# IST-DASLab/torch_cgx

Hardware: AMD Instinct MI355X
Metric: DDP samples/sec ResNet-50 4-bit (higher is better)
Workload: dtype bf16; 1 GPU; model=resnet50, global_batch=256, input=3x224x224, parallelism=dp1, backend=cgx, bits=4, bucket_size=1024, compression_active=False

## Files before the change

csrc/bindings.cc:

```cpp
#include <torch/extension.h>

#include <ATen/hip/impl/HIPStreamMasqueradingAsCUDA.h>
#include <torch/csrc/utils/pybind.h>

#include <ATen/hip/impl/HIPGuardImplMasqueradingAsCUDA.h>

#include <cstring>
#include <functional>
#include <thread>
#include <tuple>

#include "backend.h"
#include "bn_plan.h"
#include "collectives.h"
#include "conv1x1_plan.h"
#include "reducer.h"

namespace cgx {
namespace {

void run_rank_threads(int ws, int dev,
                      const std::function<void(int, hipStream_t)>& body,
                      const std::function<void()>& abort) {
  std::vector<hipStream_t> qs(ws, nullptr);
// ... 810 lines not shown
  for (int wg = 0; wg < p.grid; wg++)
    for (int tid = 0; tid < kBnThreads; tid++) {
      const BnSweep sw = bn_sweep(p, wg, tid);
      int64_t k = 0;
      for (int64_t r = sw.row; r < p.rows; r += sw.stride, k++) {
        TORCH_CHECK(k < width, "bn_sweep_indices: run longer than planned");
        o[((int64_t)wg * kBnThreads + tid) * width + k] = bn_vec(p, r, sw.cg);
      }
    }
  return out;
}

std::vector<int64_t> py_bn_partial_offsets(int64_t rows, int64_t channels,
                                           int wg) {
  const BnPlan p = bn_plan(rows, channels);
  TORCH_CHECK(p.eligible && wg >= 0 && wg < p.grid, "bn_partial_offsets: bad");
  std::vector<int64_t> offs;
  for (int tid = 0; tid < p.tc; tid++) {
    const BnSweep sw = bn_sweep(p, wg, tid);
    const int64_t o = bn_partial_offset(p, wg, sw.cg);
    for (int j = 0; j < 8; j++) offs.push_back(o + j);
  }
  return offs;
}


Conv1x1Plan conv1x1_plan_of(const at::Tensor& x, const at::Tensor& weight,
                            int64_t max_workgroups) {
  return conv1x1_plan(x.numel() / x.size(1), x.size(1), weight.size(0),
                      (int)std::min<int64_t>(max_workgroups, 1 << 20));
}

bool py_conv1x1_eligible(const at::Tensor& x, const at::Tensor& weight) {
  return bn_tensor_ok(x) && weight.is_cuda() &&
         weight.device() == x.device() &&
         weight.scalar_type() == at::kBFloat16 && weight.dim() == 4 &&
         weight.size(1) == x.size(1) && weight.size(2) == 1 &&
         weight.size(3) == 1 && weight.is_contiguous() &&
         reinterpret_cast<uintptr_t>(weight.data_ptr()) % 16 == 0 &&
         conv1x1_plan_of(x, weight, 0).eligible;
}

std::tuple<at::Tensor, at::Tensor> py_conv1x1_stats(const at::Tensor& x,
                                                    const at::Tensor& weight,
                                                    int64_t max_workgroups) {
  TORCH_CHECK(max_workgroups >= 0, "conv1x1_stats: max_workgroups >= 0");
  TORCH_CHECK(py_conv1x1_eligible(x, weight),
              "conv1x1_stats: input or weight is not eligible");
  const Conv1x1Plan p = conv1x1_plan_of(x, weight, max_workgroups);
  c10::hip::HIPGuardMasqueradingAsCUDA guard(x.device().index());
  auto y = at::empty({x.size(0), p.n, x.size(2), x.size(3)}, x.options(),
                     at::MemoryFormat::ChannelsLast);
  auto part = at::empty({p.splits, p.pstride}, x.options().dtype(at::kFloat));
  launch_conv1x1_stats(p, x.data_ptr(), weight.data_ptr(), y.data_ptr(),
                       part.data_ptr<float>(), bn_stream(x));
  return {y, part};
}

py::dict py_conv1x1_plan(int64_t rows, int64_t k, int64_t n,
                         int64_t max_workgroups) {
  const Conv1x1Plan p = conv1x1_plan(rows, k, n, (int)max_workgroups);
  py::dict d;
  d["eligible"] = p.eligible;
  d["native"] = p.native;
  d["threads"] = kConvThreads;
  d["tile_rows"] = kConvTileRows;
  d["mfma_tiles"] = p.nt;
  d["tile_channels"] = p.bn;
  d["ntiles"] = p.ntiles;
  d["k_chunk"] = p.kc;
  d["k_chunks"] = p.nchunks;
  d["resident"] = p.resident;
  d["row_tiles"] = p.row_tiles;
  d["splits"] = p.splits;
  d["grid"] = p.grid;
  d["tiles_per_split"] = p.tiles_per_split;
  d["run"] = p.run;
  d["lds_bytes"] = p.lds_bytes;
  d["partial_stride"] = p.pstride;
  d["partial_floats"] = p.partial_floats;
  return d;
}

at::Tensor py_conv1x1_walk(int64_t rows, int64_t k, int64_t n,
                           int64_t max_workgroups) {
  const Conv1x1Plan p = conv1x1_plan(rows, k, n, (int)max_workgroups);
  TORCH_CHECK(p.eligible, "conv1x1_walk: shape is not eligible");
  auto out = at::full({p.grid, p.tiles_per_split, 4}, -1,
                      at::TensorOptions().dtype(at::kLong));
  int64_t* o = out.data_ptr<int64_t>();
  for (int wg = 0; wg < p.grid; wg++) {
    const int split = conv1x1_split(p, wg), nt = conv1x1_ntile(p, wg);
    for (int i = 0; i < p.tiles_per_split; i++) {
      const int t = conv1x1_tile(p, split, i);
      if (t >= p.row_tiles) break;
      int64_t* e = o + ((int64_t)wg * p.tiles_per_split + i) * 4;
      e[0] = (int64_t)t * kConvTileRows;
      e[1] = std::min<int64_t>(e[0] + kConvTileRows, p.rows);
      e[2] = (int64_t)nt * p.bn;
      e[3] = e[2] + p.bn;
    }
  }
  return out;
}

void py_register_layer(int64_t bucket_idx, int64_t layer_idx, int64_t numel,
                       int64_t bits, int64_t bucket_size) {
  Registry::get().register_layer((int)bucket_idx, (int)layer_idx, numel,
                                 (int)bits, (int)bucket_size);
}

void py_set_bits(int64_t bucket_idx, int64_t layer_idx, int64_t bits) {
  Registry::get().set_bits((int)bucket_idx, (int)layer_idx, (int)bits);
}

void py_set_bucket(int64_t bucket_idx, int64_t layer_idx,
                   int64_t bucket_size) {
  Registry::get().set_bucket_size((int)bucket_idx, (int)layer_idx,
                                  (int)bucket_size);
}

}
}

PYBIND11_MODULE(TORCH_EXTENSION_NAME, m) {
  py::class_<cgx::ProcessGroupCGX,
             c10::intrusive_ptr<cgx::ProcessGroupCGX>, c10d::Backend>(
      m, "ProcessGroupCGX")
      .def(py::init<c10::intrusive_ptr<c10d::Store>, int, int,
                    c10::intrusive_ptr<c10d::Backend>>(),
           py::arg("store"), py::arg("rank"), py::arg("size"),
           py::arg("cpu_delegate") = nullptr);

  m.def("register_layer", &cgx::py_register_layer, py::arg("bucket_idx"),
        py::arg("layer_idx"), py::arg("layer_numel"), py::arg("bits"),
        py::arg("bucket_size"));
  m.def("set_quantization_bits", &cgx::py_set_bits);
  m.def("set_quantization_bucket_size", &cgx::py_set_bucket);
  m.def("clear_registry", [] { cgx::Registry::get().clear(); });
  m.def("registry_match",
        [](int64_t numel, int64_t key) {
          cgx::Registry::BucketInfo info;
          const bool ok = cgx::Registry::get().next(
              numel, reinterpret_cast<const void*>(key), &info);
          return py::make_tuple(ok, ok ? info.idx : -1);
        },
        py::arg("numel"), py::arg("key") = 0);
  m.def("registry_snapshot", [] {
    py::list out;
    auto& reg = cgx::Registry::get();
    for (const auto& b : reg.snapshot()) {
      py::list numels, cfgs;
      for (auto n : b.numels) numels.append(n);
      for (const auto& c : b.cfgs)
        cfgs.append(py::make_tuple(c.bits, c.bucket_size));
      out.append(py::make_tuple(b.idx, numels, cfgs));
    }
    return out;
  });

  m.def("parse_engine_config", [] {
    auto c = cgx::EngineConfig::from_env();
    py::dict d;
    d["fusion_bytes"] = c.fusion_bytes;
    d["min_elems"] = c.min_elems;
    d["default_bits"] = c.default_bits;
    d["default_bucket"] = c.default_bucket;
    d["stochastic"] = c.stochastic;
    d["inner_ring"] = c.ring;
    d["cross_ring"] = c.cross_ring;
    d["debug_a2a"] = c.debug_a2a;
    d["fake_ratio"] = c.fake_ratio;
    d["skip_incomplete"] = c.skip_incomplete;
    d["dummy"] = c.dummy;
    d["intra_compress"] = c.intra_compress;
    d["intra_broadcast"] = c.intra_broadcast;
    d["error_feedback"] = c.error_feedback;
    return d;
  });
  m.def("env_flag", &cgx::env_flag, py::arg("name"),
        py::arg("default") = false,
        "Test seam: the textual boolean parser (only \"0\" is false).");
  m.def("env_int", &cgx::env_int, py::arg("name"), py::arg("default"),
        "Test seam: the numeric parser behind the `!= 0` booleans.");
  m.def("loopback_allreduce", &cgx::py_loopback_allreduce, py::arg("buckets"),
        "Run Reducer::allreduce (flat) at world_size=len(buckets) on one GPU "
// ... 31 lines not shown
        py::arg("skip_incomplete") = false);
  m.def("dequantize_multi", &cgx::py_dequantize_multi, py::arg("comp"),
        py::arg("out"), py::arg("bits"), py::arg("bucket_size"),
        py::arg("add") = false);
  m.def("compute_topology",
        [](const c10::intrusive_ptr<c10d::Store>& store, int rank, int size,
           const std::string& hostname) {
          auto t = cgx::compute_topology(store, rank, size, hostname);
          return std::make_tuple(t.node_id, t.local_rank, t.local_size,
                                 t.n_nodes, t.uniform);
        },
        "Exchange hostnames through the store -> (node_id, local_rank, "
        "local_size, n_nodes, uniform)");
  m.def("buffer_size", &cgx::py_buffer_size, py::arg("n"), py::arg("dtype"),
        py::arg("bits"), py::arg("bucket_size"),
        py::arg("skip_incomplete") = false);
  m.def("partition", &cgx::py_partition);
  m.def("plan_bucket", &cgx::py_plan_bucket, py::arg("layer_numels"),
        py::arg("layer_cfgs"), py::arg("dtype"), py::arg("fusion_bytes"),
        py::arg("min_elems"), py::arg("fake_ratio") = 1.0,
        py::arg("dummy") = false,
        "Test seam: the bucket plan for layers laid out back to back from "
        "byte offset 0 -> (uncomp [(byte_off, count)], chunks [[(byte_off, "
        "numel, bits, bucket)]]).");
  m.def("plan_chunk", &cgx::py_plan_chunk, py::arg("views"), py::arg("dtype"),
        py::arg("ws"), py::arg("skip_incomplete") = false,
        "Test seam: the rank plan of one chunk [(byte_off, numel, bits, "
        "bucket)] -> (offs, szs, comp, rs [[(byte_off, n, bits, bucket, "
        "comp_off, skip_incomplete, fb_off)]]).");
  m.def("route_quantize", &cgx::py_route_quantize, py::arg("slices"),
        "Test seam: the launch router's quantize plan for "
        "[(in, out, fb, n, bits, bucket, skip_incomplete)] (pointers as "
        "ints) -> [(bits, kind, descs, cum, any_residual, max_gpl)].");
  m.def("route_dequantize", &cgx::py_route_dequantize, py::arg("slices"),
        py::arg("dtype"), py::arg("src_stride") = 0, py::arg("nsrc") = 1,
        py::arg("add") = false,
        "Test seam: the launch router's dequantize plan for "
        "[(in, out, n, bits, bucket, skip_incomplete)] -> "
        "[(bits, kind, descs, total_groups, any_residual)].");
  m.def("bn_act_forward", &cgx::py_bn_act_forward, py::arg("x"),
        py::arg("identity"), py::arg("weight"), py::arg("bias"),
        py::arg("running_mean"), py::arg("running_var"), py::arg("momentum"),
        py::arg("eps"), py::arg("relu"), py::arg("part") = py::none(),
        "Training-mode BatchNorm2d of a channels_last bf16 tensor, fused with "
        "an optional residual add and ReLU -> (out, mean, invstd, mask | "
        "None); updates the running statistics in place.  With `part`, the "
        "partials conv1x1_stats returned with x, the statistics pass over x "
        "is skipped.");
  m.def("bn_act_backward", &cgx::py_bn_act_backward, py::arg("dy"),
        py::arg("x"), py::arg("mean"), py::arg("invstd"), py::arg("weight"),
        py::arg("mask"), py::arg("has_identity"),
        "Backward of bn_act_forward -> (dx, dgamma, dbeta, didentity | None).");
  m.def("bn_act2_forward", &cgx::py_bn_act2_forward, py::arg("x3"),
        py::arg("xd"), py::arg("weight3"), py::arg("bias3"),
        py::arg("running_mean3"), py::arg("running_var3"),
        py::arg("momentum3"), py::arg("eps3"), py::arg("weightd"),
        py::arg("biasd"), py::arg("running_meand"), py::arg("running_vard"),
        py::arg("momentumd"), py::arg("epsd"), py::arg("relu"),
        py::arg("part3") = py::none(), py::arg("partd") = py::none(),
        "relu(bn3(x3) + bn_d(xd)) with both BatchNorms in training mode: "
        "(x3, xd, weight3, bias3, running_mean3, running_var3, momentum3, "
        "eps3, weightd, biasd, running_meand, running_vard, momentumd, epsd, "
        "relu, part3=None, partd=None) -> (out, mean3, invstd3, meand, "
        "invstdd, mask | None); part3 / partd as `part` of bn_act_forward.");
  m.def("conv1x1_stats", &cgx::py_conv1x1_stats, py::arg("x"),
        py::arg("weight"), py::arg("max_workgroups") = 0,
        "conv2d(x, weight) of a 1x1 / stride 1 / no-bias convolution on a "
        "channels_last bf16 tensor -> (y, part); part holds the per-channel "
        "(count, mean, M2) partials of y.  max_workgroups > 0 caps the "
        "persistent grid.");
  m.def("conv1x1_eligible", &cgx::py_conv1x1_eligible, py::arg("x"),
        py::arg("weight"),
        "True where conv1x1_stats takes (x, weight): CUDA, bf16, dense "
        "channels_last input, [N, K, 1, 1] weight, and a shape conv1x1_plan "
        "calls eligible.");
  m.def("conv1x1_plan", &cgx::py_conv1x1_plan, py::arg("rows"), py::arg("k"),
        py::arg("n"), py::arg("max_workgroups") = 0,
        "The launch geometry of conv1x1_stats for [rows, k] x [n, k], and "
        "`native`: whether the model uses it at this shape.");
  m.def("conv1x1_walk", &cgx::py_conv1x1_walk, py::arg("rows"), py::arg("k"),
        py::arg("n"), py::arg("max_workgroups") = 0,
        "Test seam: [grid, tiles_per_split, 4] int64, (row0, row1, n0, n1) "
        "of every tile each workgroup visits (-1: none).");
  m.def("bn_act2_backward", &cgx::py_bn_act2_backward,
        "Backward of bn_act2_forward: (dy, x3, xd, mean3, invstd3, weight3, "
        "meand, invstdd, weightd, mask) -> (dx3, dxd, dgamma3, dbeta3, "
        "dgammad, dbetad).");
  m.def("bn_act_pool_forward", &cgx::py_bn_act_pool_forward, py::arg("x"),
        py::arg("weight"), py::arg("bias"), py::arg("running_mean"),
        py::arg("running_var"), py::arg("momentum"), py::arg("eps"),
        "max_pool2d(relu(bn(x)), 3, 2, 1) in training mode -> (pooled, mean, "
        "invstd, arg); arg is one byte per pooled element.");
  m.def("bn_act_pool_backward", &cgx::py_bn_act_pool_backward, py::arg("dy"),
        py::arg("x"), py::arg("mean"), py::arg("invstd"), py::arg("weight"),
        py::arg("arg"),
        "Backward of bn_act_pool_forward -> (dx, dgamma, dbeta).");
  m.def("bn_pool_geometry", &cgx::py_bn_pool_geometry, py::arg("h"),
        py::arg("w"),
        "Test seam: (windows [oh*ow, 9], covers [h*w, 4, 2]) of the stem's "
        "3x3/2/1 pooling as the kernels index it.");
  m.def("bn_eligible", &cgx::py_bn_eligible, py::arg("x"),
        "True where the fused BatchNorm kernels take `x`: CUDA, bf16, dense "
        "channels_last, and a shape bn_plan calls eligible.");
  m.def("bn_plan", &cgx::py_bn_plan, py::arg("rows"), py::arg("channels"),
        "Test seam: the launch geometry of the fused BatchNorm kernels for a "
        "[rows, channels] activation.");
  m.def("bn_sweep_indices", &cgx::py_bn_sweep_indices, py::arg("rows"),
        py::arg("channels"),
        "Test seam: [grid*threads, rows_per_thread+1] int64, the 16-byte "
        "vector indices every thread visits (-1: none).");
  m.def("bn_partial_offsets", &cgx::py_bn_partial_offsets, py::arg("rows"),
        py::arg("channels"), py::arg("wg"),
        "Test seam: the partial-buffer floats workgroup `wg` writes.");
  m.attr("FLAG_SKIP_INCOMPLETE") = cgx::kFlagSkipIncomplete;
  m.attr("FLAG_TAIL_ONLY") = cgx::kFlagTailOnly;
  m.attr("KIND_FAST") = (int)cgx::kFast;
  m.attr("KIND_GENERIC") = (int)cgx::kGeneric;
  m.attr("KIND_TWO_PASS") = (int)cgx::kTwoPass;
  m.attr("KIND_SUB") = (int)cgx::kSub;
}
```

csrc/conv1x1_kernels.hip:

```cpp
#include <hip/hip_runtime.h>

#include "bn_moments.h"
#include "check.h"
#include "conv1x1_plan.h"

namespace cgx {
namespace {

constexpr int kT = kConvThreads;

typedef __bf16 bf16x8 __attribute__((ext_vector_type(8)));
typedef __bf16 bf16x2 __attribute__((ext_vector_type(2)));
typedef float f32x2 __attribute__((ext_vector_type(2)));
typedef float f32x16 __attribute__((ext_vector_type(16)));

template <int KC>
__device__ inline int w_slot(int n, int q) {
  return n * (KC / 8) + (q ^ (KC == 64 ? (n >> 1) & 7 : n & 15));
}

__device__ inline int acc_row(int i, int h) {
  return (i & 3) + 8 * (i >> 2) + 4 * h;
}

// ... 105 lines not shown
      if (acc_row(2 * e + 1, h) < live) st.push(hi);
    }

    const int odd = c & 1;
#pragma unroll
    for (int jp = 0; jp < NT / 2; jp++) {
#pragma unroll
      for (int jj = 0; jj < 2; jj++)
#pragma unroll
        for (int e = 0; e < 8; e++) {
          const unsigned own = pk[2 * jp + jj][e];
          const unsigned other = (unsigned)__builtin_amdgcn_update_dpp(
              0, (int)own, 0xB1, 0xf, 0xf, false);
          const unsigned word = odd ? (other >> 16) | (own & 0xffff0000u)
                                    : (own & 0xffffu) | (other << 16);
          const int row = acc_row(2 * e, h) + odd;
          stage32[row * 32 + ((jj * 16 + (c >> 1)) ^ ((row & 1) << 4))] = word;
        }
      asm volatile("" ::: "memory");
      __builtin_amdgcn_wave_barrier();
#pragma unroll
      for (int u = 0; u < 4; u++) {
        const int idx = u * 64 + lane, row = idx >> 3, q = idx & 7;
        const uint4 v = stage[row * 8 + (q ^ ((row & 1) << 2))];
        if (row < live) y[(r0 + row) * nvec + (n0 + jp * 64) / 8 + q] = v;
      }
      asm volatile("" ::: "memory");
      __builtin_amdgcn_wave_barrier();
    }
  }

  __syncthreads();
  float* sc = reinterpret_cast<float*>(lds);
  const int run = wave * 2 + h;
#pragma unroll
  for (int j = 0; j < NT; j++) {
    sc[run * BN + j * 32 + c] = st.mean[j];
    sc[(8 + run) * BN + j * 32 + c] = st.m2[j];
  }
  if (c == 0) sc[16 * BN + run] = st.n;
  __syncthreads();
  if (tid < BN) {
    Moments<1> m[8];
#pragma unroll
    for (int r = 0; r < 8; r++) {
      m[r].n = sc[16 * BN + r];
      m[r].mean[0] = sc[r * BN + tid];
      m[r].m2[0] = sc[(8 + r) * BN + tid];
    }
#pragma unroll
    for (int step = 1; step < 8; step *= 2)
#pragma unroll
      for (int r = 0; r < 8; r += 2 * step)
        m[r].merge(m[r + step].n, m[r + step].mean, m[r + step].m2);
    float* row = part + (int64_t)split * p.pstride;
    row[n0 + tid] = m[0].mean[0];
    row[p.n + n0 + tid] = m[0].m2[0];
    if (tid == 0) row[2 * p.n + ntile] = m[0].n;
  }
}

template <int NT, int KC, bool RES>
void launch(const Conv1x1Plan& p, const void* x, const void* w, void* y,
            float* part, hipStream_t stream) {
  static const hipError_t attr = hipFuncSetAttribute(
      reinterpret_cast<const void*>(&conv1x1_stats<NT, KC, RES>),
      hipFuncAttributeMaxDynamicSharedMemorySize,
      kConvWLdsBytes + kConvStageBytes);
  CGX_HIP_CHECK(attr);
  hipLaunchKernelGGL((conv1x1_stats<NT, KC, RES>), dim3(p.grid), dim3(kT),
                     p.lds_bytes, stream, static_cast<const uint4*>(x),
                     static_cast<const uint4*>(w), static_cast<uint4*>(y), part,
                     p);
}

template <int NT>
void launch_nt(const Conv1x1Plan& p, const void* x, const void* w, void* y,
               float* part, hipStream_t stream) {
  if (p.kc == 64) launch<NT, 64, true>(p, x, w, y, part, stream);
  else if (p.resident) launch<NT, 128, true>(p, x, w, y, part, stream);
  else launch<NT, 128, false>(p, x, w, y, part, stream);
}

}

void launch_conv1x1_stats(const Conv1x1Plan& p, const void* x, const void* w,
                          void* y, float* part, hipStream_t stream) {
  TORCH_CHECK(p.eligible, "conv1x1_stats: shape is not eligible");
  if (p.nt == 2) launch_nt<2>(p, x, w, y, part, stream);
  else if (p.nt == 4) launch_nt<4>(p, x, w, y, part, stream);
  else launch_nt<8>(p, x, w, y, part, stream);
  CGX_HIP_CHECK(hipGetLastError());
}

}
```

csrc/conv1x1_plan.cc:

```cpp
#include "conv1x1_plan.h"

#include <algorithm>

namespace cgx {
namespace {

struct Measured {
  int k, n;
  int64_t rows;
};
constexpr Measured kNative[] = {
    {64, 64, 802816},   {64, 256, 802816},  {256, 64, 802816},
    {256, 128, 802816}, {128, 512, 200704}, {512, 128, 200704},
    {256, 1024, 50176},
};

bool measured_faster(int64_t rows, int k, int n) {
  for (const Measured& m : kNative)
    if (m.k == k && m.n == n && m.rows == rows) return true;
  return false;
}

bool pow2_in(int64_t v, int64_t lo, int64_t hi) {
  return v >= lo && v <= hi && (v & (v - 1)) == 0;
}

}

Conv1x1Plan conv1x1_plan(int64_t rows, int64_t k, int64_t n,
                         int max_workgroups) {
  Conv1x1Plan p;
  p.rows = rows;
  p.eligible = pow2_in(k, 64, 2048) && pow2_in(n, 64, 2048) && rows >= 2 &&
               rows <= kBnMaxRows;
  if (!p.eligible) return p;
  p.k = (int)k;
  p.n = (int)n;
  p.native = measured_faster(rows, p.k, p.n);

  p.nt = std::min(p.n / 32, kConvMaxNt);
  p.bn = 32 * p.nt;
  p.ntiles = p.n / p.bn;
  p.kc = p.k == 64 ? 64 : 128;
  p.nchunks = p.k / p.kc;
  p.resident = p.bn * p.k * 2 <= kConvWLdsBytes;
  p.lds_bytes = p.bn * (p.resident ? p.k : p.kc) * 2 + kConvStageBytes;

  p.row_tiles = (int)((rows + kConvTileRows - 1) / kConvTileRows);
  const int by_regs = p.nt == 8 ? 1 : p.nt == 4 ? 2 : 3;
  const int per_cu = std::max(1, std::min(kConvLdsBytes / p.lds_bytes, by_regs));
  int64_t splits = std::min<int64_t>(
      p.row_tiles, std::max(1, kConvCus * per_cu / p.ntiles));
  splits = std::min(splits, std::max<int64_t>(1, rows / 82));
  if (max_workgroups > 0)
    splits = std::min<int64_t>(splits, std::max(1, max_workgroups / p.ntiles));
  p.splits = (int)splits;
  p.grid = p.ntiles * p.splits;
  p.tiles_per_split = (p.row_tiles + p.splits - 1) / p.splits;
  p.run = 16 * p.tiles_per_split;
  p.pstride = 2 * p.n + p.ntiles;
  p.partial_floats = (int64_t)p.splits * p.pstride;
  return p;
}

}
```

csrc/conv1x1_plan.h:

```cpp
#pragma once

#include <cstdint>

#include "bn_plan.h"

namespace cgx {

constexpr int kConvThreads = 256;
constexpr int kConvTileRows = 128;
constexpr int kConvMaxNt = 8;
constexpr int kConvCus = 256;
constexpr int kConvLdsBytes = 160 * 1024;
constexpr int kConvWLdsBytes = 128 * 1024;
constexpr int kConvStageBytes = 16 * 1024;

struct Conv1x1Plan {
  int64_t rows = 0;
  int k = 0, n = 0;
  bool eligible = false;
  bool native = false;
  int nt = 0;
  int bn = 0;
  int ntiles = 0;
  int kc = 0;
  int nchunks = 0;
  bool resident = false;
  int row_tiles = 0;
  int splits = 0;
  int grid = 0;
  int tiles_per_split = 0;
  int run = 0;
  int lds_bytes = 0;
  int pstride = 0;
  int64_t partial_floats = 0;
};

Conv1x1Plan conv1x1_plan(int64_t rows, int64_t k, int64_t n,
                         int max_workgroups = 0);

__host__ __device__ inline int conv1x1_ntile(const Conv1x1Plan& p, int wg) {
  return wg % p.ntiles;
}
__host__ __device__ inline int conv1x1_split(const Conv1x1Plan& p, int wg) {
  return wg / p.ntiles;
}
__host__ __device__ inline int conv1x1_tile(const Conv1x1Plan& p, int split,
                                            int i) {
  return split + i * p.splits;
}

inline BnPartials conv1x1_partials(const float* part, int n, int splits,
                                   int ntiles) {
  BnPartials q;
  q.mean = part;
  q.m2 = part + n;
  q.cnt = part + 2 * n;
  q.channels = n;
  q.splits = splits;
  q.tc = n / ntiles / 8;
  q.pstride = q.cstride = 2 * n + ntiles;
  return q;
}

void launch_conv1x1_stats(const Conv1x1Plan& p, const void* x, const void* w,
                          void* y, float* part, hipStream_t stream);

}
```

torch_cgx_amd/models/resnet.py:

```python

from __future__ import annotations

import torch
import torch.nn as nn

from ..ops.fused_bn import bn_act, bn_act_pool, conv_bn_act


class Bottleneck(nn.Module):
    expansion = 4

    def __init__(self, inplanes: int, planes: int, stride: int = 1,
                 downsample: nn.Module = None):
        super().__init__()
        self.conv1 = nn.Conv2d(inplanes, planes, 1, bias=False)
        self.bn1 = nn.BatchNorm2d(planes)
        self.conv2 = nn.Conv2d(planes, planes, 3, stride=stride, padding=1,
                               bias=False)
        self.bn2 = nn.BatchNorm2d(planes)
        self.conv3 = nn.Conv2d(planes, planes * self.expansion, 1, bias=False)
        self.bn3 = nn.BatchNorm2d(planes * self.expansion)
        self.relu = nn.ReLU(inplace=True)
        self.downsample = downsample
        self.stride = stride

    def forward(self, x):
        identity = x
        out = conv_bn_act(self.conv1, self.bn1, x)
        out = bn_act(self.bn2, self.conv2(out))
        if self.downsample is not None:
            conv, bn = self.downsample[0], self.downsample[1]
            return conv_bn_act(self.conv3, self.bn3, out, identity,
                               identity_conv=conv, identity_bn=bn)
        return conv_bn_act(self.conv3, self.bn3, out, identity)


class ResNet(nn.Module):
    def __init__(self, layers, num_classes: int = 1000):
        super().__init__()
        self.inplanes = 64
        self.conv1 = nn.Conv2d(3, 64, 7, stride=2, padding=3, bias=False)
        self.bn1 = nn.BatchNorm2d(64)
        self.relu = nn.ReLU(inplace=True)
        self.maxpool = nn.MaxPool2d(3, stride=2, padding=1)
        self.layer1 = self._make_layer(64, layers[0])
        self.layer2 = self._make_layer(128, layers[1], stride=2)
        self.layer3 = self._make_layer(256, layers[2], stride=2)
        self.layer4 = self._make_layer(512, layers[3], stride=2)
        self.avgpool = nn.AdaptiveAvgPool2d(1)
        self.fc = nn.Linear(512 * Bottleneck.expansion, num_classes)
        for m in self.modules():
            if isinstance(m, nn.Conv2d):
                nn.init.kaiming_normal_(m.weight, mode="fan_out",
                                        nonlinearity="relu")
            elif isinstance(m, nn.BatchNorm2d):
                nn.init.constant_(m.weight, 1)
                nn.init.constant_(m.bias, 0)

    def _make_layer(self, planes: int, blocks: int, stride: int = 1):
        downsample = None
        if stride != 1 or self.inplanes != planes * Bottleneck.expansion:
            downsample = nn.Sequential(
                nn.Conv2d(self.inplanes, planes * Bottleneck.expansion, 1,
                          stride=stride, bias=False),
                nn.BatchNorm2d(planes * Bottleneck.expansion),
            )
        layers = [Bottleneck(self.inplanes, planes, stride, downsample)]
        self.inplanes = planes * Bottleneck.expansion
        for _ in range(1, blocks):
            layers.append(Bottleneck(self.inplanes, planes))
        return nn.Sequential(*layers)

    def forward(self, x):
        x = bn_act_pool(self.bn1, self.conv1(x), self.maxpool)
        x = self.layer4(self.layer3(self.layer2(self.layer1(x))))
        x = self.avgpool(x).flatten(1)
        return self.fc(x)


def resnet50(num_classes: int = 1000) -> ResNet:
    return ResNet([3, 4, 6, 3], num_classes)


def resnet18(num_classes: int = 1000) -> nn.Module:

    class BasicBlock(nn.Module):
        def __init__(self, inp, planes, stride=1, down=None):
            super().__init__()
            self.c1 = nn.Conv2d(inp, planes, 3, stride, 1, bias=False)
            self.b1 = nn.BatchNorm2d(planes)
            self.c2 = nn.Conv2d(planes, planes, 3, 1, 1, bias=False)
            self.b2 = nn.BatchNorm2d(planes)
            self.down = down

        def forward(self, x):
            idt = x if self.down is None else self.down(x)
            out = torch.relu(self.b1(self.c1(x)))
            return torch.relu(self.b2(self.c2(out)) + idt)

    class R18(nn.Module):
        def __init__(self):
            super().__init__()
            self.stem = nn.Sequential(
                nn.Conv2d(3, 64, 7, 2, 3, bias=False), nn.BatchNorm2d(64),
                nn.ReLU(inplace=True), nn.MaxPool2d(3, 2, 1))
            chans = [64, 128, 256, 512]
            blocks = []
            inp = 64
            for i, c in enumerate(chans):
                stride = 1 if i == 0 else 2
                down = None
# ... 17 lines not shown
```

torch_cgx_amd/ops/fused_bn.py:

```python

from __future__ import annotations

import os

import torch
import torch.nn.functional as F

from .. import _C


class _BnAct(torch.autograd.Function):
    @staticmethod
    def forward(ctx, x, identity, weight, bias, running_mean, running_var,
                momentum, eps, relu, part):
        out, mean, invstd, mask = _C.bn_act_forward(
            x, identity, weight, bias, running_mean, running_var, momentum,
            eps, relu, part)
        ctx.save_for_backward(x, mean, invstd, weight, mask)
        ctx.has_identity = identity is not None
        return out

    @staticmethod
    def backward(ctx, dy):
        x, mean, invstd, weight, mask = ctx.saved_tensors
# ... 32 lines not shown
                eps):
        out, mean, invstd, arg = _C.bn_act_pool_forward(
            x, weight, bias, running_mean, running_var, momentum, eps)
        ctx.save_for_backward(x, mean, invstd, weight, arg)
        return out

    @staticmethod
    def backward(ctx, dy):
        x, mean, invstd, weight, arg = ctx.saved_tensors
        dx, dgamma, dbeta = _C.bn_act_pool_backward(dy, x, mean, invstd,
                                                    weight, arg)
        return (dx, dgamma, dbeta, None, None, None, None)


def fused_bn_enabled() -> bool:
    return os.environ.get("CGX_FUSED_BN", "1") != "0"


def _native(bn, x, identity) -> bool:
    if not (bn.training and bn.track_running_stats
            and bn.momentum is not None and fused_bn_enabled()):
        return False
    if bn.weight is None or bn.bias is None:
        return False
    if not (x.is_cuda and _C.bn_eligible(x)):
        return False
    if identity is not None and not (
            identity.shape == x.shape and identity.device == x.device
            and _C.bn_eligible(identity)):
        return False
    return bn.weight.dtype == torch.float32


def _bn_args(bn):
    return (bn.weight, bn.bias, bn.running_mean, bn.running_var, bn.momentum,
            bn.eps)


def bn_act(bn: torch.nn.BatchNorm2d, x: torch.Tensor,
           identity: torch.Tensor = None, relu: bool = True,
           identity_bn: torch.nn.BatchNorm2d = None,
           part: torch.Tensor = None,
           identity_part: torch.Tensor = None) -> torch.Tensor:
    if identity_bn is not None:
        if _native(bn, x, identity) and _native(identity_bn, identity, x):
            bn.num_batches_tracked.add_(1)
            identity_bn.num_batches_tracked.add_(1)
            return _BnActJoin.apply(x, identity, *_bn_args(bn),
                                    *_bn_args(identity_bn), relu, part,
                                    identity_part)
        out = bn(x) + identity_bn(identity)
        return F.relu(out, inplace=True) if relu else out
    if _native(bn, x, identity):
        bn.num_batches_tracked.add_(1)
        return _BnAct.apply(x, identity, *_bn_args(bn), relu, part)
    out = bn(x)
    if identity is not None:
        out = out + identity
    if relu:
        out = F.relu(out, inplace=True)
    return out


class _Conv1x1Stats(torch.autograd.Function):

    @staticmethod
    @torch.amp.custom_fwd(device_type="cuda", cast_inputs=torch.bfloat16)
    def forward(ctx, x, weight):
        y, part = _C.conv1x1_stats(x, weight)
        ctx.save_for_backward(x, weight)
        ctx.mark_non_differentiable(part)
        return y, part

    @staticmethod
    @torch.amp.custom_bwd(device_type="cuda")
    def backward(ctx, dy, _dpart):
        x, weight = ctx.saved_tensors
        dx, dw, _ = torch.ops.aten.convolution_backward(
            dy, x, weight, None, (1, 1), (0, 0), (1, 1), False, (0, 0), 1,
            (ctx.needs_input_grad[0], ctx.needs_input_grad[1], False))
        return dx, dw


def native_conv1x1_mode() -> str:
    if not fused_bn_enabled():
        return "0"
    return os.environ.get("CGX_NATIVE_CONV1X1", "1")


def _conv1x1_native(conv, bn, x) -> bool:
    mode = native_conv1x1_mode()
    if mode == "0":
        return False
    if not (type(conv) is torch.nn.Conv2d and conv.kernel_size == (1, 1)
            and conv.stride == (1, 1) and conv.padding == (0, 0)
            and conv.dilation == (1, 1) and conv.groups == 1
            and conv.bias is None and conv.padding_mode == "zeros"):
        return False
    if not (bn.training and bn.track_running_stats
            and bn.momentum is not None and bn.weight is not None
            and bn.bias is not None and bn.weight.dtype == torch.float32):
        return False
    if not (x.is_cuda and x.dim() == 4 and x.dtype == torch.bfloat16
            and _C.bn_eligible(x)):
        return False
    w = conv.weight
    autocast = (torch.is_autocast_enabled("cuda")
                and torch.get_autocast_dtype("cuda") == torch.bfloat16)
    if not (w.device == x.device and w.shape[1] == x.shape[1]
            and (w.dtype == torch.bfloat16
                 or (autocast and w.dtype == torch.float32))):
        return False
    if w.dtype == torch.bfloat16 and not _C.conv1x1_eligible(x, w):
        return False
    plan = _C.conv1x1_plan(x.numel() // x.shape[1], x.shape[1], w.shape[0])
    return plan["eligible"] and (plan["native"] or mode == "all")


def _conv(conv, bn, x):
    if _conv1x1_native(conv, bn, x):
        return _Conv1x1Stats.apply(x, conv.weight)
    return conv(x), None


def conv_bn_act(conv: torch.nn.Conv2d, bn: torch.nn.BatchNorm2d,
                x: torch.Tensor, identity: torch.Tensor = None,
                relu: bool = True, identity_conv: torch.nn.Conv2d = None,
                identity_bn: torch.nn.BatchNorm2d = None) -> torch.Tensor:
    y, part = _conv(conv, bn, x)
    if identity_conv is None:
        return bn_act(bn, y, identity, relu, part=part)
    yd, partd = _conv(identity_conv, identity_bn, identity)
    return bn_act(bn, y, yd, relu, identity_bn=identity_bn, part=part,
                  identity_part=partd)


def _pool_is_3x3_s2_p1(pool) -> bool:
    def pair(v):
        return tuple(v) if isinstance(v, (tuple, list)) else (v, v)

    return (type(pool) is torch.nn.MaxPool2d
            and pair(pool.kernel_size) == (3, 3) and pair(pool.stride) == (2, 2)
            and pair(pool.padding) == (1, 1) and pair(pool.dilation) == (1, 1)
            and not pool.ceil_mode and not pool.return_indices)


def bn_act_pool(bn: torch.nn.BatchNorm2d, x: torch.Tensor,
                pool: torch.nn.Module) -> torch.Tensor:
    if _pool_is_3x3_s2_p1(pool) and _native(bn, x, None):
        bn.num_batches_tracked.add_(1)
        return _BnActPool.apply(x, *_bn_args(bn))
    return pool(bn_act(bn, x))
```

Baseline: 7660 samples/s.

## Add native 1x1 conv backward-data kernel fusing residual gradient add

Adds a HIP MFMA kernel computing the input gradient of 1x1 stride-1 convolutions, with weights transposed into LDS, and optionally adds the residual skip gradient before a single bf16 rounding. The Bottleneck block now forks its identity through a custom autograd function, so the skip gradient enters the conv backward directly instead of through a separate add. Weight gradients still use aten. The native path is enabled only for a hardcoded table of ResNet-50 shapes, and it risks being slower than the vendor library on other shapes.

```diff
diff --git a/csrc/bindings.cc b/csrc/bindings.cc
--- a/csrc/bindings.cc
+++ b/csrc/bindings.cc
@@ -916,10 +916,7 @@
   return d;
 }
 
-at::Tensor py_conv1x1_walk(int64_t rows, int64_t k, int64_t n,
-                           int64_t max_workgroups) {
-  const Conv1x1Plan p = conv1x1_plan(rows, k, n, (int)max_workgroups);
-  TORCH_CHECK(p.eligible, "conv1x1_walk: shape is not eligible");
+at::Tensor conv1x1_walk_of(const Conv1x1Plan& p) {
   auto out = at::full({p.grid, p.tiles_per_split, 4}, -1,
                       at::TensorOptions().dtype(at::kLong));
   int64_t* o = out.data_ptr<int64_t>();
@@ -936,6 +933,87 @@
     }
   }
   return out;
+}
+
+at::Tensor py_conv1x1_walk(int64_t rows, int64_t k, int64_t n,
+                           int64_t max_workgroups) {
+  const Conv1x1Plan p = conv1x1_plan(rows, k, n, (int)max_workgroups);
+  TORCH_CHECK(p.eligible, "conv1x1_walk: shape is not eligible");
+  return conv1x1_walk_of(p);
+}
+
+
+int clamp_workgroups(int64_t max_workgroups) {
+  return (int)std::min<int64_t>(max_workgroups, 1 << 20);
+}
+
+bool py_conv1x1_bwd_eligible(const at::Tensor& dy, const at::Tensor& weight,
+                             const c10::optional<at::Tensor>& skip) {
+  if (!(bn_tensor_ok(dy) && weight.is_cuda() &&
+        weight.device() == dy.device() &&
+        weight.scalar_type() == at::kBFloat16 && weight.dim() == 4 &&
+        weight.size(0) == dy.size(1) && weight.size(2) == 1 &&
+        weight.size(3) == 1 && weight.is_contiguous() &&
+        reinterpret_cast<uintptr_t>(weight.data_ptr()) % 16 == 0 &&
+        conv1x1_bwd_plan(dy.numel() / dy.size(1), weight.size(1),
+                         weight.size(0), skip.has_value())
+            .eligible))
+    return false;
+  if (!skip.has_value()) return true;
+  const at::Tensor& s = *skip;
+  return s.dim() == 4 && s.size(0) == dy.size(0) &&
+         s.size(1) == weight.size(1) && s.size(2) == dy.size(2) &&
+         s.size(3) == dy.size(3) && s.device() == dy.device() &&
+         bn_tensor_ok(s);
+}
+
+at::Tensor py_conv1x1_bwd_data(const at::Tensor& dy, const at::Tensor& weight,
+                               const c10::optional<at::Tensor>& skip,
+                               int64_t max_workgroups) {
+  TORCH_CHECK(max_workgroups >= 0, "conv1x1_bwd_data: max_workgroups >= 0");
+  TORCH_CHECK(py_conv1x1_bwd_eligible(dy, weight, skip),
+              "conv1x1_bwd_data: dy, weight or skip is not eligible");
+  const Conv1x1Plan p = conv1x1_bwd_plan(
+      dy.numel() / dy.size(1), weight.size(1), weight.size(0),
+      skip.has_value(), clamp_workgroups(max_workgroups));
+  c10::hip::HIPGuardMasqueradingAsCUDA guard(dy.device().index());
+  auto dx = at::empty({dy.size(0), p.n, dy.size(2), dy.size(3)}, dy.options(),
+                      at::MemoryFormat::ChannelsLast);
+  launch_conv1x1_bwd_data(p, dy.data_ptr(), weight.data_ptr(),
+                          skip.has_value() ? skip->data_ptr() : nullptr,
+                          dx.data_ptr(), bn_stream(dy));
+  return dx;
+}
+
+py::dict py_conv1x1_bwd_plan(int64_t rows, int64_t k, int64_t n, bool with_add,
+                             int64_t max_workgroups) {
+  const Conv1x1Plan p =
+      conv1x1_bwd_plan(rows, k, n, with_add, clamp_workgroups(max_workgroups));
+  py::dict d;
+  d["eligible"] = p.eligible;
+  d["native"] = p.native;
+  d["threads"] = kConvThreads;
+  d["tile_rows"] = kConvTileRows;
+  d["mfma_tiles"] = p.nt;
+  d["tile_channels"] = p.bn;
+  d["ntiles"] = p.ntiles;
+  d["k_chunk"] = p.kc;
+  d["k_chunks"] = p.nchunks;
+  d["resident"] = p.resident;
+  d["row_tiles"] = p.row_tiles;
+  d["splits"] = p.splits;
+  d["grid"] = p.grid;
+  d["tiles_per_split"] = p.tiles_per_split;
+  d["lds_bytes"] = p.lds_bytes;
+  return d;
+}
+
+at::Tensor py_conv1x1_bwd_walk(int64_t rows, int64_t k, int64_t n,
+                               bool with_add, int64_t max_workgroups) {
+  const Conv1x1Plan p =
+      conv1x1_bwd_plan(rows, k, n, with_add, clamp_workgroups(max_workgroups));
+  TORCH_CHECK(p.eligible, "conv1x1_bwd_walk: shape is not eligible");
+  return conv1x1_walk_of(p);
 }
 
 void py_register_layer(int64_t bucket_idx, int64_t layer_idx, int64_t numel,
@@ -1133,6 +1211,26 @@
         py::arg("n"), py::arg("max_workgroups") = 0,
         "Test seam: [grid, tiles_per_split, 4] int64, (row0, row1, n0, n1) "
         "of every tile each workgroup visits (-1: none).");
+  m.def("conv1x1_bwd_data", &cgx::py_conv1x1_bwd_data, py::arg("dy"),
+        py::arg("weight"), py::arg("skip") = py::none(),
+        py::arg("max_workgroups") = 0,
+        "Input gradient of conv2d(x, weight) for a 1x1 / stride 1 convolution "
+        "on channels_last bf16 tensors, plus `skip` (a bf16 channels_last "
+        "tensor of dx's shape) where given: dx = bf16(dy * W + skip), rounded "
+        "once.  `skip` is not written.");
+  m.def("conv1x1_bwd_eligible", &cgx::py_conv1x1_bwd_eligible, py::arg("dy"),
+        py::arg("weight"), py::arg("skip") = py::none(),
+        "True where conv1x1_bwd_data takes (dy, weight, skip).");
+  m.def("conv1x1_bwd_plan", &cgx::py_conv1x1_bwd_plan, py::arg("rows"),
+        py::arg("k"), py::arg("n"), py::arg("with_add") = false,
+        py::arg("max_workgroups") = 0,
+        "The launch geometry of conv1x1_bwd_data for dx [rows, k] from dy "
+        "[rows, n], and `native`: whether the model uses it for this problem.");
+  m.def("conv1x1_bwd_walk", &cgx::py_conv1x1_bwd_walk, py::arg("rows"),
+        py::arg("k"), py::arg("n"), py::arg("with_add") = false,
+        py::arg("max_workgroups") = 0,
+        "Test seam: conv1x1_walk for the plan of conv1x1_bwd_plan; channels "
+        "are dx's.");
   m.def("bn_act2_backward", &cgx::py_bn_act2_backward,
         "Backward of bn_act2_forward: (dy, x3, xd, mean3, invstd3, weight3, "
         "meand, invstdd, weightd, mask) -> (dx3, dxd, dgamma3, dbeta3, "
diff --git a/csrc/conv1x1_kernels.hip b/csrc/conv1x1_kernels.hip
--- a/csrc/conv1x1_kernels.hip
+++ b/csrc/conv1x1_kernels.hip
@@ -211,6 +211,198 @@
   else launch<NT, 128, false>(p, x, w, y, part, stream);
 }
 
+
+template <int NT, int KC>
+__device__ inline void stage_wt(uint4* dst, const uint4* __restrict__ w, int k0,
+                                int kw, int chunk, int tid) {
+  constexpr int kblocks = 4 * NT;
+  for (int idx = tid; idx < kblocks * (KC / 8); idx += kT) {
+    const int n8 = (idx & 7) + 8 * (idx / (8 * kblocks));
+    const int k8 = (idx >> 3) % kblocks;
+    unsigned r[8][4];
+#pragma unroll
+    for (int i = 0; i < 8; i++) {
+      const uint4 v =
+          w[((int64_t)(chunk * KC + n8 * 8 + i) * kw + k0) / 8 + k8];
+      r[i][0] = v.x, r[i][1] = v.y, r[i][2] = v.z, r[i][3] = v.w;
+    }
+#pragma unroll
+    for (int kk = 0; kk < 8; kk++) {
+      unsigned o[4];
+#pragma unroll
+      for (int m = 0; m < 4; m++) {
+        const unsigned a = r[2 * m][kk >> 1], b = r[2 * m + 1][kk >> 1];
+        o[m] = kk & 1 ? (a >> 16) | (b & 0xffff0000u)
+                      : (a & 0xffffu) | (b << 16);
+      }
+      dst[w_slot<KC>(k8 * 8 + kk, n8)] = make_uint4(o[0], o[1], o[2], o[3]);
+    }
+  }
+}
+
+template <int NT, int KC, bool RES, bool ADD>
+__global__ __launch_bounds__(kT) void conv1x1_bwd_data(
+    const uint4* __restrict__ dy, const uint4* __restrict__ w,
+    const uint4* __restrict__ skip, uint4* __restrict__ dx, Conv1x1Plan p) {
+  extern __shared__ uint4 lds[];
+  constexpr int BN = 32 * NT, cpr = KC / 8, steps = KC / 16;
+  constexpr int wchunks = BN * cpr;
+  const int tid = threadIdx.x, wave = tid >> 6, lane = tid & 63;
+  const int c = lane & 31, h = lane >> 5;
+  const int split = conv1x1_split(p, blockIdx.x);
+  const int n0 = conv1x1_ntile(p, blockIdx.x) * BN;
+  const int kvec = p.k / 8, nvec = p.n / 8;
+  uint4* stage = lds + (RES ? p.nchunks : 1) * wchunks + wave * 512;
+  float* stagef = reinterpret_cast<float*>(stage);
+
+  if (RES) {
+    for (int kc = 0; kc < p.nchunks; kc++)
+      stage_wt<NT, KC>(lds + kc * wchunks, w, n0, p.n, kc, tid);
+    __syncthreads();
+  }
+
+  auto a_row = [&](int t) {
+    int64_t r = (int64_t)t * kConvTileRows + wave * 32 + c;
+    r = r < p.rows ? r : p.rows - 1;
+    return dy + r * kvec;
+  };
+
+  uint4 a[steps], an[steps];
+  const uint4* xr = a_row(split);
+#pragma unroll
+  for (int s = 0; s < steps; s++) a[s] = xr[2 * s + h];
+
+  for (int i = 0; i < p.tiles_per_split; i++) {
+    const int t = conv1x1_tile(p, split, i);
+    if (t >= p.row_tiles) break;
+    const int tn = conv1x1_tile(p, split, i + 1);
+    const uint4* xn = a_row(tn < p.row_tiles ? tn : t);
+
+    f32x16 acc[NT];
+#pragma unroll
+    for (int j = 0; j < NT; j++)
+#pragma unroll
+      for (int e = 0; e < 16; e++) acc[j][e] = 0.f;
+
+    for (int kc = 0; kc < p.nchunks; kc++) {
+      const uint4* src = kc + 1 < p.nchunks ? xr + (kc + 1) * cpr : xn;
+#pragma unroll
+      for (int s = 0; s < steps; s++) an[s] = src[2 * s + h];
+      if (!RES) {
+        __syncthreads();
+        stage_wt<NT, KC>(lds, w, n0, p.n, kc, tid);
+        __syncthreads();
+      }
+      const uint4* wl = lds + (RES ? kc * wchunks : 0);
+#pragma unroll
+      for (int s = 0; s < steps; s++) {
+        const bf16x8 av = __builtin_bit_cast(bf16x8, a[s]);
+#pragma unroll
+        for (int j = 0; j < NT; j++) {
+          const uint4 b = wl[w_slot<KC>(j * 32 + c, 2 * s + h)];
+          acc[j] = __builtin_amdgcn_mfma_f32_32x32x16_bf16(
+              av, __builtin_bit_cast(bf16x8, b), acc[j], 0, 0, 0);
+        }
+      }
+#pragma unroll
+      for (int s = 0; s < steps; s++) a[s] = an[s];
+    }
+    xr = xn;
+
+    const int64_t r0 = (int64_t)t * kConvTileRows + wave * 32;
+    const int live = (int)(p.rows - r0 < 32 ? p.rows - r0 : 32);
+
+#pragma unroll
+    for (int jp = 0; jp < NT / 2; jp++) {
+      uint4 sk[4];
+      if (ADD) {
+#pragma unroll
+        for (int u = 0; u < 4; u++) {
+          const int idx = u * 64 + lane, row = idx >> 3, q = idx & 7;
+          sk[u] = make_uint4(0, 0, 0, 0);
+          if (row < live)
+            sk[u] = skip[(r0 + row) * nvec + (n0 + jp * 64) / 8 + q];
+        }
+      }
+#pragma unroll
+      for (int jj = 0; jj < 2; jj++)
+#pragma unroll
+        for (int e = 0; e < 16; e++) {
+          const int row = acc_row(e, h);
+          stagef[row * 64 + ((jj * 32 + c) ^ ((row & 1) << 2))] =
+              acc[2 * jp + jj][e];
+        }
+      asm volatile("" ::: "memory");
+      __builtin_amdgcn_wave_barrier();
+#pragma unroll
+      for (int u = 0; u < 4; u++) {
+        const int idx = u * 64 + lane, row = idx >> 3, q = idx & 7;
+        const uint4 lo = stage[row * 16 + 2 * q + (row & 1)];
+        const uint4 hi = stage[row * 16 + 2 * q + ((row & 1) ^ 1)];
+        float f[8] = {__uint_as_float(lo.x), __uint_as_float(lo.y),
+                      __uint_as_float(lo.z), __uint_as_float(lo.w),
+                      __uint_as_float(hi.x), __uint_as_float(hi.y),
+                      __uint_as_float(hi.z), __uint_as_float(hi.w)};
+        if (ADD) {
+          const unsigned s4[4] = {sk[u].x, sk[u].y, sk[u].z, sk[u].w};
+#pragma unroll
+          for (int m = 0; m < 4; m++) {
+            f[2 * m] += __uint_as_float(s4[m] << 16);
+            f[2 * m + 1] += __uint_as_float(s4[m] & 0xffff0000u);
+          }
+        }
+        const uint4 v = make_uint4(pack_bf16(f[0], f[1]), pack_bf16(f[2], f[3]),
+                                   pack_bf16(f[4], f[5]), pack_bf16(f[6], f[7]));
+        if (row < live) dx[(r0 + row) * nvec + (n0 + jp * 64) / 8 + q] = v;
+      }
+      asm volatile("" ::: "memory");
+      __builtin_amdgcn_wave_barrier();
+    }
+  }
+}
+
+template <int NT, int KC, bool RES, bool ADD>
+void launch_bwd(const Conv1x1Plan& p, const void* dy, const void* w,
+                const void* skip, void* dx, hipStream_t stream) {
+  static const hipError_t attr = hipFuncSetAttribute(
+      reinterpret_cast<const void*>(&conv1x1_bwd_data<NT, KC, RES, ADD>),
+      hipFuncAttributeMaxDynamicSharedMemorySize,
+      kConvWLdsBytes + kConvBwdStageBytes);
+  CGX_HIP_CHECK(attr);
+  hipLaunchKernelGGL((conv1x1_bwd_data<NT, KC, RES, ADD>), dim3(p.grid),
+                     dim3(kT), p.lds_bytes, stream,
+                     static_cast<const uint4*>(dy),
+                     static_cast<const uint4*>(w),
+                     static_cast<const uint4*>(skip), static_cast<uint4*>(dx),
+                     p);
+}
+
+template <int NT, bool ADD>
+void launch_bwd_nt(const Conv1x1Plan& p, const void* dy, const void* w,
+                   const void* skip, void* dx, hipStream_t stream) {
+  if (p.kc == 64) launch_bwd<NT, 64, true, ADD>(p, dy, w, skip, dx, stream);
+  else if (p.resident)
+    launch_bwd<NT, 128, true, ADD>(p, dy, w, skip, dx, stream);
+  else launch_bwd<NT, 128, false, ADD>(p, dy, w, skip, dx, stream);
+}
+
+template <bool ADD>
+void launch_bwd_add(const Conv1x1Plan& p, const void* dy, const void* w,
+                    const void* skip, void* dx, hipStream_t stream) {
+  if (p.nt == 2) launch_bwd_nt<2, ADD>(p, dy, w, skip, dx, stream);
+  else if (p.nt == 4) launch_bwd_nt<4, ADD>(p, dy, w, skip, dx, stream);
+  else launch_bwd_nt<8, ADD>(p, dy, w, skip, dx, stream);
+}
+
+}
+
+void launch_conv1x1_bwd_data(const Conv1x1Plan& p, const void* dy,
+                             const void* w, const void* skip, void* dx,
+                             hipStream_t stream) {
+  TORCH_CHECK(p.eligible, "conv1x1_bwd_data: shape is not eligible");
+  if (skip) launch_bwd_add<true>(p, dy, w, skip, dx, stream);
+  else launch_bwd_add<false>(p, dy, w, skip, dx, stream);
+  CGX_HIP_CHECK(hipGetLastError());
 }
 
 void launch_conv1x1_stats(const Conv1x1Plan& p, const void* x, const void* w,
diff --git a/csrc/conv1x1_plan.cc b/csrc/conv1x1_plan.cc
--- a/csrc/conv1x1_plan.cc
+++ b/csrc/conv1x1_plan.cc
@@ -25,6 +25,50 @@
   return v >= lo && v <= hi && (v & (v - 1)) == 0;
 }
 
+struct MeasuredBwd {
+  int k, n;
+  int64_t rows;
+  bool with_add;
+};
+constexpr MeasuredBwd kNativeBwd[] = {
+    {64, 64, 802816, true},    {256, 64, 802816, true},
+    {256, 128, 802816, true},  {512, 128, 200704, true},
+    {512, 256, 200704, true},  {1024, 256, 50176, true},
+    {64, 256, 802816, false},  {128, 512, 200704, false},
+};
+
+bool measured_faster_bwd(int64_t rows, int k, int n, bool with_add) {
+  for (const MeasuredBwd& m : kNativeBwd)
+    if (m.k == k && m.n == n && m.rows == rows && m.with_add == with_add)
+      return true;
+  return false;
+}
+
+void tile_geometry(Conv1x1Plan& p, int stage_bytes) {
+  p.nt = std::min(p.n / 32, kConvMaxNt);
+  p.bn = 32 * p.nt;
+  p.ntiles = p.n / p.bn;
+  p.kc = p.k == 64 ? 64 : 128;
+  p.nchunks = p.k / p.kc;
+  p.resident = p.bn * p.k * 2 <= kConvWLdsBytes;
+  p.lds_bytes = p.bn * (p.resident ? p.k : p.kc) * 2 + stage_bytes;
+  p.row_tiles = (int)((p.rows + kConvTileRows - 1) / kConvTileRows);
+}
+
+int64_t splits_by_occupancy(const Conv1x1Plan& p, int by_regs) {
+  const int per_cu = std::max(1, std::min(kConvLdsBytes / p.lds_bytes, by_regs));
+  return std::min<int64_t>(p.row_tiles,
+                           std::max(1, kConvCus * per_cu / p.ntiles));
+}
+
+void set_grid(Conv1x1Plan& p, int64_t splits, int max_workgroups) {
+  if (max_workgroups > 0)
+    splits = std::min<int64_t>(splits, std::max(1, max_workgroups / p.ntiles));
+  p.splits = (int)splits;
+  p.grid = p.ntiles * p.splits;
+  p.tiles_per_split = (p.row_tiles + p.splits - 1) / p.splits;
+}
+
 }
 
 Conv1x1Plan conv1x1_plan(int64_t rows, int64_t k, int64_t n,
@@ -37,30 +81,33 @@
   p.k = (int)k;
   p.n = (int)n;
   p.native = measured_faster(rows, p.k, p.n);
-
-  p.nt = std::min(p.n / 32, kConvMaxNt);
-  p.bn = 32 * p.nt;
-  p.ntiles = p.n / p.bn;
-  p.kc = p.k == 64 ? 64 : 128;
-  p.nchunks = p.k / p.kc;
-  p.resident = p.bn * p.k * 2 <= kConvWLdsBytes;
-  p.lds_bytes = p.bn * (p.resident ? p.k : p.kc) * 2 + kConvStageBytes;
-
-  p.row_tiles = (int)((rows + kConvTileRows - 1) / kConvTileRows);
+  tile_geometry(p, kConvStageBytes);
   const int by_regs = p.nt == 8 ? 1 : p.nt == 4 ? 2 : 3;
-  const int per_cu = std::max(1, std::min(kConvLdsBytes / p.lds_bytes, by_regs));
-  int64_t splits = std::min<int64_t>(
-      p.row_tiles, std::max(1, kConvCus * per_cu / p.ntiles));
-  splits = std::min(splits, std::max<int64_t>(1, rows / 82));
-  if (max_workgroups > 0)
-    splits = std::min<int64_t>(splits, std::max(1, max_workgroups / p.ntiles));
-  p.splits = (int)splits;
-  p.grid = p.ntiles * p.splits;
-  p.tiles_per_split = (p.row_tiles + p.splits - 1) / p.splits;
+  set_grid(p,
+           std::min(splits_by_occupancy(p, by_regs),
+                    std::max<int64_t>(1, rows / 82)),
+           max_workgroups);
   p.run = 16 * p.tiles_per_split;
   p.pstride = 2 * p.n + p.ntiles;
   p.partial_floats = (int64_t)p.splits * p.pstride;
   return p;
 }
 
+Conv1x1Plan conv1x1_bwd_plan(int64_t rows, int64_t k, int64_t n, bool with_add,
+                             int max_workgroups) {
+  Conv1x1Plan p;
+  p.rows = rows;
+  p.eligible = pow2_in(k, 64, 2048) && pow2_in(n, 64, 2048) && rows >= 2 &&
+               rows <= kBnMaxRows;
+  if (!p.eligible) return p;
+  p.k = (int)n;
+  p.n = (int)k;
+  p.native = measured_faster_bwd(rows, (int)k, (int)n, with_add);
+  tile_geometry(p, kConvBwdStageBytes);
+  const int by_regs = p.resident ? (p.nt == 8 ? 2 : p.nt == 4 ? 3 : 4)
+                                 : (p.nt == 8 ? 1 : 2);
+  set_grid(p, splits_by_occupancy(p, by_regs), max_workgroups);
+  return p;
 }
+
+}
diff --git a/csrc/conv1x1_plan.h b/csrc/conv1x1_plan.h
--- a/csrc/conv1x1_plan.h
+++ b/csrc/conv1x1_plan.h
@@ -13,6 +13,7 @@
 constexpr int kConvLdsBytes = 160 * 1024;
 constexpr int kConvWLdsBytes = 128 * 1024;
 constexpr int kConvStageBytes = 16 * 1024;
+constexpr int kConvBwdStageBytes = 32 * 1024;
 
 struct Conv1x1Plan {
   int64_t rows = 0;
@@ -37,6 +38,9 @@
 
 Conv1x1Plan conv1x1_plan(int64_t rows, int64_t k, int64_t n,
                          int max_workgroups = 0);
+
+Conv1x1Plan conv1x1_bwd_plan(int64_t rows, int64_t k, int64_t n, bool with_add,
+                             int max_workgroups = 0);
 
 __host__ __device__ inline int conv1x1_ntile(const Conv1x1Plan& p, int wg) {
   return wg % p.ntiles;
@@ -65,4 +69,8 @@
 void launch_conv1x1_stats(const Conv1x1Plan& p, const void* x, const void* w,
                           void* y, float* part, hipStream_t stream);
 
+void launch_conv1x1_bwd_data(const Conv1x1Plan& p, const void* dy,
+                             const void* w, const void* skip, void* dx,
+                             hipStream_t stream);
+
 }
diff --git a/torch_cgx_amd/models/resnet.py b/torch_cgx_amd/models/resnet.py
--- a/torch_cgx_amd/models/resnet.py
+++ b/torch_cgx_amd/models/resnet.py
@@ -4,7 +4,8 @@
 import torch
 import torch.nn as nn
 
-from ..ops.fused_bn import bn_act, bn_act_pool, conv_bn_act
+from ..ops.fused_bn import (bn_act, bn_act_pool, conv_bn_act,
+                            conv_bn_act_fork)
 
 
 class Bottleneck(nn.Module):
@@ -25,8 +26,7 @@
         self.stride = stride
 
     def forward(self, x):
-        identity = x
-        out = conv_bn_act(self.conv1, self.bn1, x)
+        out, identity = conv_bn_act_fork(self.conv1, self.bn1, x)
         out = bn_act(self.bn2, self.conv2(out))
         if self.downsample is not None:
             conv, bn = self.downsample[0], self.downsample[1]
diff --git a/torch_cgx_amd/ops/fused_bn.py b/torch_cgx_amd/ops/fused_bn.py
--- a/torch_cgx_amd/ops/fused_bn.py
+++ b/torch_cgx_amd/ops/fused_bn.py
@@ -138,57 +138,132 @@
         return dx, dw
 
 
+class _Conv1x1Fork(torch.autograd.Function):
+
+    @staticmethod
+    @torch.amp.custom_fwd(device_type="cuda", cast_inputs=torch.bfloat16)
+    def forward(ctx, x, weight, native_fwd, fork):
+        if native_fwd:
+            y, part = _C.conv1x1_stats(x, weight)
+            ctx.mark_non_differentiable(part)
+        else:
+            y, part = F.conv2d(x, weight), None
+        ctx.save_for_backward(x, weight)
+        ctx.set_materialize_grads(False)
+        return y, part, (x.view_as(x) if fork else None)
+
+    @staticmethod
+    @torch.amp.custom_bwd(device_type="cuda")
+    def backward(ctx, dy, _dpart, dskip):
+        x, weight = ctx.saved_tensors
+        dx = dw = None
+        if dy is not None and ctx.needs_input_grad[1]:
+            dw = _conv1x1_backward(dy, x, weight, (False, True, False))[1]
+        if ctx.needs_input_grad[0]:
+            dx = dskip if dy is None else _conv1x1_dx(dy, x, weight, dskip)
+        return dx, dw, None, None
+
+
+def _conv1x1_backward(dy, x, weight, mask):
+    return torch.ops.aten.convolution_backward(
+        dy, x, weight, None, (1, 1), (0, 0), (1, 1), False, (0, 0), 1, mask)
+
+
+def _conv1x1_dx(dy, x, weight, dskip):
+    mode = native_conv1x1_bwd_mode()
+    if mode != "0" and _C.conv1x1_bwd_eligible(dy, weight, dskip):
+        plan = _C.conv1x1_bwd_plan(x.numel() // x.shape[1], x.shape[1],
+                                   weight.shape[0], dskip is not None)
+        if plan["native"] or mode == "all":
+            return _C.conv1x1_bwd_data(dy, weight, dskip)
+    dx = _conv1x1_backward(dy, x, weight, (True, False, False))[0]
+    return dx if dskip is None else dx + dskip
+
+
 def native_conv1x1_mode() -> str:
     if not fused_bn_enabled():
         return "0"
     return os.environ.get("CGX_NATIVE_CONV1X1", "1")
 
 
-def _conv1x1_native(conv, bn, x) -> bool:
-    mode = native_conv1x1_mode()
-    if mode == "0":
-        return False
+def native_conv1x1_bwd_mode() -> str:
+    if native_conv1x1_mode() == "0":
+        return "0"
+    return os.environ.get("CGX_NATIVE_CONV1X1_BWD", "1")
+
+
+def _conv1x1_shape(conv, bn, x):
+    if native_conv1x1_mode() == "0":
+        return None
     if not (type(conv) is torch.nn.Conv2d and conv.kernel_size == (1, 1)
             and conv.stride == (1, 1) and conv.padding == (0, 0)
             and conv.dilation == (1, 1) and conv.groups == 1
             and conv.bias is None and conv.padding_mode == "zeros"):
-        return False
+        return None
     if not (bn.training and bn.track_running_stats
             and bn.momentum is not None and bn.weight is not None
             and bn.bias is not None and bn.weight.dtype == torch.float32):
-        return False
+        return None
     if not (x.is_cuda and x.dim() == 4 and x.dtype == torch.bfloat16
             and _C.bn_eligible(x)):
-        return False
+        return None
     w = conv.weight
     autocast = (torch.is_autocast_enabled("cuda")
                 and torch.get_autocast_dtype("cuda") == torch.bfloat16)
     if not (w.device == x.device and w.shape[1] == x.shape[1]
             and (w.dtype == torch.bfloat16
                  or (autocast and w.dtype == torch.float32))):
-        return False
+        return None
     if w.dtype == torch.bfloat16 and not _C.conv1x1_eligible(x, w):
-        return False
-    plan = _C.conv1x1_plan(x.numel() // x.shape[1], x.shape[1], w.shape[0])
+        return None
+    return x.numel() // x.shape[1], x.shape[1], w.shape[0]
+
+
+def _conv1x1_native(shape) -> bool:
+    plan = _C.conv1x1_plan(*shape)
+    return plan["eligible"] and (plan["native"]
+                                 or native_conv1x1_mode() == "all")
+
+
+def _conv1x1_bwd_native(shape, with_add) -> bool:
+    mode = native_conv1x1_bwd_mode()
+    if mode == "0":
+        return False
+    plan = _C.conv1x1_bwd_plan(*shape, with_add)
     return plan["eligible"] and (plan["native"] or mode == "all")
 
 
-def _conv(conv, bn, x):
-    if _conv1x1_native(conv, bn, x):
-        return _Conv1x1Stats.apply(x, conv.weight)
-    return conv(x), None
+def _conv(conv, bn, x, fork=False):
+    shape = _conv1x1_shape(conv, bn, x)
+    if shape is None:
+        return conv(x), None, x
+    fwd = _conv1x1_native(shape)
+    if torch.is_grad_enabled():
+        fork = fork and _conv1x1_bwd_native(shape, True)
+        if fork or _conv1x1_bwd_native(shape, False):
+            y, part, skip = _Conv1x1Fork.apply(x, conv.weight, fwd, fork)
+            return y, part, (skip if fork else x)
+    if fwd:
+        return _Conv1x1Stats.apply(x, conv.weight) + (x,)
+    return conv(x), None, x
 
 
 def conv_bn_act(conv: torch.nn.Conv2d, bn: torch.nn.BatchNorm2d,
                 x: torch.Tensor, identity: torch.Tensor = None,
                 relu: bool = True, identity_conv: torch.nn.Conv2d = None,
                 identity_bn: torch.nn.BatchNorm2d = None) -> torch.Tensor:
-    y, part = _conv(conv, bn, x)
+    y, part, _ = _conv(conv, bn, x)
     if identity_conv is None:
         return bn_act(bn, y, identity, relu, part=part)
-    yd, partd = _conv(identity_conv, identity_bn, identity)
+    yd, partd, _ = _conv(identity_conv, identity_bn, identity)
     return bn_act(bn, y, yd, relu, identity_bn=identity_bn, part=part,
                   identity_part=partd)
+
+
+def conv_bn_act_fork(conv: torch.nn.Conv2d, bn: torch.nn.BatchNorm2d,
+                     x: torch.Tensor, relu: bool = True):
+    y, part, skip = _conv(conv, bn, x, fork=True)
+    return bn_act(bn, y, None, relu, part=part), skip
 
 
 def _pool_is_3x3_s2_p1(pool) -> bool:
```

After: 7993 samples/s, median of 6. 1.04x the previous value.
